# mkshing/e4t-diffusion

Measured on AMD Instinct MI355X. Metric: E4T pretrain images/sec @512px bf16, higher is better.
Workload: dtype bf16

## Files before the change

### e4t-diffusion_amd/csrc/gemm.hip

```cpp
#include "gemm_common.h"

#ifndef E4T_GEMM_PS_DEFAULT
#define E4T_GEMM_PS_DEFAULT 0
#endif
extern "C" __attribute__((visibility("hidden"))) int e4t_launch_gemm_ps(const GemmArgs* p, int conv, int bn, int general, int ncu, hipStream_t st);

namespace {


template <int BM, int BN, int WGM, int WGN, int MODE>
__global__ __launch_bounds__(256) void gemm_kernel(GemmArgs p) {
  constexpr int WM = BM / WGM, WN = BN / WGN;
  constexpr int FM = WM / 32, FN = WN / 32;
  constexpr int NA = BM * (BK / 8) / 256;
  constexpr int NB = BN * (BK / 8) / 256;
  static_assert(WGM * WGN == 4, "4 waves per workgroup");
  static_assert(NA >= 1 && NB >= 1, "tile too small");

  __shared__ __attribute__((aligned(16))) bf16_t smem[(BM + BN) * LDS_LD];
  bf16_t* const As = smem;
  bf16_t* const Bs = smem + BM * LDS_LD;

  const int tid = threadIdx.x;
  const int lane = tid & 63, wave = tid >> 6;
// ... 1033 lines not shown
#pragma unroll
    for (int ks = 0; ks < 2; ++ks)
#pragma unroll
      for (int i = 0; i < 2; ++i)
#pragma unroll
        for (int j = 0; j < 2; ++j)
          acc[mh * 2 + i][j] = __builtin_amdgcn_mfma_f32_32x32x16_bf16(af[i][ks], bfr[j][ks], acc[mh * 2 + i][j], 0, 0, 0);
    __builtin_amdgcn_s_setprio(0);
    __builtin_amdgcn_sched_barrier(0);
    __builtin_amdgcn_s_barrier();
    __builtin_amdgcn_sched_barrier(0);
  };
  auto ktile = [&](auto Bc, auto KXc, auto SPc, auto ALLc, int kt) __attribute__((always_inline)) {
    phase(Bc, I0{}, ALLc, KXc, SPc, kt); phase(Bc, I1{}, ALLc, KXc, SPc, kt); phase(Bc, I2{}, ALLc, KXc, SPc, kt); phase(Bc, I3{}, ALLc, KXc, SPc, kt);
  };

  if (wr == 1) __builtin_amdgcn_s_barrier();
  {
    using YES = std::true_type; using NO = std::false_type;
    int kt = kt_begin;
    for (; kt + 8 <= kt_end; kt += 6) {
      ktile(I0{}, I0{}, I0{}, YES{}, kt);     ktile(I1{}, I1{}, I0{}, YES{}, kt + 1); ktile(I0{}, I2{}, I0{}, YES{}, kt + 2);
      ktile(I1{}, I0{}, I1{}, YES{}, kt + 3); ktile(I0{}, I1{}, I1{}, YES{}, kt + 4); ktile(I1{}, I2{}, I1{}, YES{}, kt + 5);
    }
    if (kt < kt_end) { ktile(I0{}, I0{}, I0{}, NO{}, kt); ktile(I1{}, I1{}, I0{}, NO{}, kt + 1); ktile(I0{}, I2{}, I0{}, NO{}, kt + 2); kt += 3; }
    if (kt < kt_end) { ktile(I1{}, I0{}, I1{}, NO{}, kt); ktile(I0{}, I1{}, I1{}, NO{}, kt + 1); ktile(I1{}, I2{}, I1{}, NO{}, kt + 2); kt += 3; }
  }
  if (wr == 0) __builtin_amdgcn_s_barrier();
  __syncthreads();
  write_tile<64, 64, 2, 2, GENERAL>(p, *(f32x16(*)[2][2])(acc + 0), wave_stage<64, 64>(smem, wave), lane, m0 + wr * 128, n0 + wc * 64);
  __syncthreads();
  write_tile<64, 64, 2, 2, GENERAL>(p, *(f32x16(*)[2][2])(acc + 2), wave_stage<64, 64>(smem, wave), lane, m0 + wr * 128 + 64, n0 + wc * 64);
}
static bool conv_pps_ok(const GemmArgs& p, int batch) {
  static const bool on = CONV_STRIP && getenv("E4T_CONV_NOSTRIP") == nullptr;
  const bool rows = p.Win % 256 == 0 || (p.Win >= 16 && 256 % p.Win == 0 && p.Hin % (256 / p.Win) == 0);
  return on && p.mode == E4T_CONV_S1 && p.chan_major && batch == 1 && rows && p.Wout == p.Win && p.Hout == p.Hin && p.Cin % 64 == 0 &&
         p.K == 9 * p.Cin && p.ktiles_per_split % 3 == 0 && p.M % 256 == 0;
}

template <int MODE, int BN, bool GENERAL>
__global__ __launch_bounds__(512) void gemm_pq_kernel(GemmArgs p) {
  constexpr int BM = 256, HK = 32;
  constexpr int WR = BN == 320 ? 4 : 2, WC = 8 / WR;
  constexpr int WM = BM / WR, WN = BN / WC;
  constexpr int FM = WM / 32, FN = WN / 32;
  constexpr int QA = BM * HK, QB = BN * HK;
  constexpr int HALF = QA + QB, BUF = 2 * HALF;
  constexpr int NBP = BN / 16;
  constexpr int NBJ = (NBP + 7) / 8;
  constexpr int NBLAST = NBP - 8 * (NBJ - 1);
  constexpr int ESTG = 8 * 32 * (WN + 8);
  static_assert(BN == 256 || BN == 320, "tile width");
  static_assert(2 * BUF * 2 <= 160 * 1024 && ESTG <= 2 * BUF, "LDS budget");
  __shared__ __attribute__((aligned(16))) bf16_t smem[2 * BUF];

  const int tid = threadIdx.x;
  const int lane = tid & 63, wave = __builtin_amdgcn_readfirstlane(tid >> 6);
  const int grp = wave >> 2;
  const int wr = wave / WC, wc = wave % WC;
  int tile_x, tile_y;
  xcd_tile(tile_x, tile_y, p.group_m);
  int m0 = tile_y * BM;
  const int n0 = tile_x * BN;
  const int mrows = p.M - m0;
  if (p.panel_rows) m0 = (m0 / p.panel_rows) * p.panel_stride + p.panel_off + m0 % p.panel_rows;

// ... 203 lines not shown
    __builtin_amdgcn_sched_barrier(0);
  };
  using I0 = std::integral_constant<int, 0>; using I1 = std::integral_constant<int, 1>;
  using I2 = std::integral_constant<int, 2>; using I3 = std::integral_constant<int, 3>;

  if (grp == 1) __builtin_amdgcn_s_barrier();
  {
    int kt = kt_begin;
    for (; kt + 2 <= kt_end; kt += 2) {
      phase(I0{}, I0{}, kt); phase(I0{}, I1{}, kt); phase(I0{}, I2{}, kt); phase(I0{}, I3{}, kt);
      phase(I1{}, I0{}, kt + 1); phase(I1{}, I1{}, kt + 1); phase(I1{}, I2{}, kt + 1); phase(I1{}, I3{}, kt + 1);
    }
    if (kt < kt_end) { phase(I0{}, I0{}, kt); phase(I0{}, I1{}, kt); phase(I0{}, I2{}, kt); phase(I0{}, I3{}, kt); }
  }
  if (grp == 0) __builtin_amdgcn_s_barrier();
  __syncthreads();
  if (p.panel_rows) p.M = m0 + min(mrows, BM);
  auto slice = [&](auto Ic) {
    constexpr int i = decltype(Ic)::value;
    write_tile<32, WN, 1, FN, GENERAL>(p, *(f32x16(*)[1][FN])(&acc[i][0]), wave_stage<32, WN>(smem, wave), lane, m0 + wr * WM + i * 32, n0 + wc * WN);
  };
  slice(I0{});
  __syncthreads();
  slice(I1{});
  if constexpr (FM == 4) {
    __syncthreads();
    slice(I2{});
    __syncthreads();
    slice(I3{});
  }
  if constexpr (MODE == 0) {
    if (p.tail_rows) gemm_tail<8, GENERAL>(p, (float*)smem, wave, lane);
  }
}

#ifdef E4T_EXPERIMENTAL
template <int MODE>
__global__ __launch_bounds__(512) void gemm_pt_kernel(GemmArgs p) {
  constexpr int BM = 512, BN = 128, HK = 32;
  constexpr int QA = BM * HK, QB = BN * HK;
  constexpr int HALF = QA + QB;
  constexpr int SMEM = 4 * HALF;
  static_assert(8 * 64 * (64 + 8) <= SMEM, "epilogue staging must fit");
  __shared__ __attribute__((aligned(16))) bf16_t smem[SMEM];

  const int tid = threadIdx.x;
  const int lane = tid & 63, wave = __builtin_amdgcn_readfirstlane(tid >> 6);
  const int wr = wave >> 2, wc = wave & 3;
  int tile_x, tile_y;
  xcd_tile(tile_x, tile_y, p.group_m);
  const int m0 = tile_y * BM, n0 = tile_x * BN;

  const int nkt = p.K / BK;
  const int bz = blockIdx.z / p.splitk, sz = blockIdx.z - bz * p.splitk;
  p.A += bz * p.strideA;
  if (p.A2) p.A2 += bz * p.strideA;
  p.B += bz * p.strideB;
  if (p.bias) p.bias += bz * p.strideBias;
  if (!p.reduce_batch) {
    if (p.flags & E4T_OUT_F32) p.C = (float*)p.C + bz * p.strideC;
    else p.C = (bf16_t*)p.C + bz * p.strideC;
  }
  const int kt_begin = sz * p.ktiles_per_split;
  int kt_end = kt_begin + p.ktiles_per_split;
  if (kt_end > nkt) kt_end = nkt;

// ... 355 lines not shown
    for (int k = 0; k < 8; ++k) {
      float x = v[k] * p.alpha + bi[k] + rb[k];
      if (p.flags & E4T_ACT_GELU) x = gelu_f(x);
      v[k] = x + rs[k];
    }
    *(uint4*)((bf16_t*)p.C + (size_t)row * p.ldc + c8) = pack8(v);
  }
}

__global__ __launch_bounds__(256) void splitk_reduce4f_kernel(GemmArgs p, int nz) {
  const int n4 = p.N >> 2;
  const size_t total = (size_t)p.M * p.N, total4 = (size_t)p.M * n4;
  const int bz = blockIdx.y;
  float* Cf = (float*)p.C + (p.reduce_batch ? 0 : bz * p.strideC);
  const float* ws = p.ws + (size_t)bz * nz * total;
  for (size_t i4 = (size_t)blockIdx.x * 256 + threadIdx.x; i4 < total4; i4 += (size_t)gridDim.x * 256) {
    const int row = (int)(i4 / n4), c4 = (int)(i4 - (size_t)row * n4) * 4;
    const size_t idx = (size_t)row * p.N + c4;
    float4 v = make_float4(0.f, 0.f, 0.f, 0.f);
    for (int z0 = 0; z0 < nz; z0 += 8) {
      float4 t[8];
#pragma unroll
      for (int u = 0; u < 8; ++u) t[u] = *(const float4*)(ws + (size_t)min(z0 + u, nz - 1) * total + idx);
#pragma unroll
      for (int u = 0; u < 8; ++u) {
        const float w = z0 + u < nz ? 1.f : 0.f;
        v.x += t[u].x * w; v.y += t[u].y * w; v.z += t[u].z * w; v.w += t[u].w * w;
      }
    }
    float4* c = (float4*)(Cf + (size_t)row * p.ldc + c4);
    float4 o = make_float4(v.x * p.alpha, v.y * p.alpha, v.z * p.alpha, v.w * p.alpha);
    if (p.flags & E4T_ACCUM) { const float4 a = *c; o.x += a.x; o.y += a.y; o.z += a.z; o.w += a.w; }
    *c = o;
  }
}

struct GemmPlan {
  int tile;
  int stages;
  bool kt32;
  bool general_epi;
  bool buf_ok;
  int tm, tn, gx, gy;
  int splitk, ktiles_per_split;
  unsigned a_bytes, a2_bytes, b_bytes;
};

int device_cu_count() {
  static int ncu = [] {
    int dev = 0, n = 0;
    if (hipGetDevice(&dev) != hipSuccess || hipDeviceGetAttribute(&n, hipDeviceAttributeMultiprocessorCount, dev) != hipSuccess || n <= 0) n = 256;
    return n;
  }();
  return ncu;
}

bool ps_rounds_ok(long long units, int ncu) {
  if (units < ncu) return false;
  const long long rounds = (units + ncu - 1) / ncu;
  return units * 100 >= rounds * ncu * 85;
}

struct SmallGridPlan { int tile, stages, splitk; };
struct SmallGridCand { int tile, stages, tm, tn, occ; float t1, tk, epi; bool general_ok; };
SmallGridPlan small_grid_plan(int M, int N, int nkt, bool conv, bool general, int splitk_req, bool wants_colstats, int ncu) {
  static const SmallGridCand cands[] = {
// ... 1 lines not shown
      {128, 2, 128, 128, 2, 0.875f, 0.544f, 1.08f, true}, {128, 4, 128, 128, 1, 0.596f, 0.544f, 1.08f, false},
      {160, 2, 128, 160, 2, 0.955f, 0.629f, 3.41f, false}, {160, 3, 128, 160, 1, 0.861f, 0.629f, 3.41f, false}};
  static const int splits[] = {1, 2, 3, 4, 6, 8, 12};
  const float launch = 1.6f, pro = 0.945f, red0 = 4.49f, red_bytes_per_us = 4.05e6f, conv_mul = 0.916f, stats_pass = 6.0f;
  SmallGridPlan best = {128, 2, 1};
  float best_t = 1e30f;
  for (const SmallGridCand& c : cands) {
    if (general && !c.general_ok) continue;
    if (c.tile == 160 && N % 160 != 0) continue;
    for (int sk : splits) {
      if (splitk_req > 0 && sk != 1) continue;
      const int s = splitk_req > 0 ? (splitk_req < nkt ? splitk_req : nkt) : sk;
      if (s > 1 && splitk_req <= 0 && (nkt / s < 4 || (double)M * N * s * 4.0 > 256e6)) continue;
      const int kps = cdiv(nkt, s);
      const long long wgs = (long long)cdiv(M, c.tm) * cdiv(N, c.tn) * s;
      const long long per_cu = cdivl(wgs, ncu);
      const long long q = per_cu / c.occ, r = per_cu % c.occ;
      const float full = c.occ > 1 ? c.occ * c.tk : c.t1;
      const float rem = r == 0 ? 0.f : (r == 1 ? c.t1 : (float)r * c.tk);
      float per_kt = (float)q * full + rem;
      if (conv) per_kt *= conv_mul;
      const float rounds = (float)cdivl(per_cu, c.occ);
      float t = launch + rounds * (pro + c.epi) + (float)kps * per_kt;
      if (s > 1) {
        t += red0 + ((float)s * 4.f + 2.f) * (float)M * (float)N / red_bytes_per_us + rounds * c.epi * 0.5f;
        if (wants_colstats) t += stats_pass;
      }
      if (t < best_t) { best_t = t; best = {c.tile, c.stages, s}; }
    }
  }
  return best;
}

GemmPlan plan_gemm(const GemmArgs& p, bool conv, int tile_hint, int splitk_req, int batch) {
  GemmPlan pl;
  const int nkt = cdiv(p.K, BK);
  int stages = 2;
  int model_splitk = 0;
  bool kt32 = false;
  if (tile_hint >= 3000 && tile_hint < 5000) { stages = tile_hint / 1000; tile_hint %= 1000; }
  else if (tile_hint >= 5000 && tile_hint < 6000) { kt32 = true; stages = 4; tile_hint %= 1000; }
  int tile = tile_hint;
#ifndef E4T_EXPERIMENTAL
  if (kt32 && tile != 256) { kt32 = false; stages = 2; }
  if (tile != 64 && tile != 128 && tile != 160) stages = 2;
  if (tile == 256 && !kt32) { kt32 = true; stages = 3; }
  if (tile == 640) tile = 128;
  if (tile == 1128) tile = 128;
  if (tile == 1160) tile = 160;
#endif
  static const bool allow256 = getenv("E4T_GEMM_REGSTAGE") == nullptr;
#ifdef E4T_EXPERIMENTAL
  static const bool auto256 = getenv("E4T_GEMM_AUTO256") != nullptr;
#else
  const bool auto256 = false;
#endif
  const bool r2_rules = false;
  const bool whole_k = p.K % BK == 0 && (!p.A2 || p.K1 % BK == 0);
  const bool ps_ok = allow256 && whole_k && batch == 1 && !p.reduce_batch && splitk_req <= 1;
  if (tile != 64 && tile != 128 && tile != 256 && tile != 160 && tile != 512 && tile != 640 && tile != 1128 && tile != 1160 && tile != 2320) {
    const long long t256 = (long long)cdiv(p.M, 256) * cdiv(p.N, 128) * batch;
    const long long t128 = (long long)cdiv(p.M, 128) * cdiv(p.N, 128) * batch;
    tile = (allow256 && auto256 && t256 >= 256) ? 256 : (t128 >= 256 || (nkt >= 32 && t128 >= 64)) ? 128 : 64;
    if (allow256 && tile == 128 && p.N % 160 == 0 && p.N <= 960 && (long long)cdiv(p.M, 128) * (p.N / 160) * batch >= 128) tile = 160;
    const bool no_pp = false;
    const long long tpp = (long long)cdiv(p.M, 256) * (p.N / 256) * batch;
    if (allow256 && !no_pp && tile == 128 && p.N % 256 == 0 && whole_k && nkt >= (conv ? 16 : (r2_rules ? 32 : 20)) && tpp >= 512) tile = 512;
    if (allow256 && !no_pp && tile == 128 && p.N % 256 == 0 && whole_k && nkt >= 128 && tpp >= 64 && tpp < (r2_rules ? 512 : 256)) tile = 512;
    if (!r2_rules && allow256 && !no_pp && tile == 128 && p.N % 256 == 0 && whole_k && nkt >= 20 && tpp >= 224 && tpp <= 256) tile = 512;
#ifdef E4T_EXPERIMENTAL
    static const bool auto_pt = getenv("E4T_GEMM_PT") != nullptr;
#else
    const bool auto_pt = false;
#endif
    if (auto_pt && allow256 && tile == 128 && p.N % 128 == 0 && p.N % 256 != 0 && p.K % BK == 0 && nkt >= 16 && !p.A2 &&
        (long long)cdiv(p.M, 512) * (p.N / 128) * batch >= 512) tile = 640;
    const bool general = (p.flags & E4T_ACT_GELU) || (p.rowbias && p.rows_per_batch % 32 != 0);
    if (!r2_rules && allow256 && tile == 128 && !general && p.N % 160 == 0 && p.N > 960 && nkt >= 20 &&
        (long long)cdiv(p.M, 128) * (p.N / 160) * batch >= 1024) tile = 160;
    if (!r2_rules && allow256 && tile == 128 && !general && (p.N % 128 == 0 || p.N < 128) &&
        (long long)cdiv(p.M, 256) * cdiv(p.N, 128) * batch >= 768) { tile = 256; kt32 = true; stages = 3; }
    const bool no_pq = false;
    if (!r2_rules && !no_pq && allow256 && batch == 1 && (!general || !conv) && whole_k && p.N % 320 == 0) {
      const long long t320 = (long long)cdiv(p.M, 256) * (p.N / 320);
      const int ncu = device_cu_count();
      const double eff = (double)t320 / (double)(cdivl(t320, ncu) * ncu);
      if (t320 >= ncu && ((nkt >= 20 && eff >= 0.75) || (nkt >= 10 && eff >= 0.99) || (nkt >= 5 && p.N == 320 && eff >= 0.99))) {
        tile = 2320; kt32 = false; stages = 2;
      }
    }
#ifdef E4T_EXPERIMENTAL
    static const int auto_ps = getenv("E4T_GEMM_PS") ? atoi(getenv("E4T_GEMM_PS")) : E4T_GEMM_PS_DEFAULT;
#else
    const int auto_ps = 0;
#endif
    if (auto_ps && ps_ok && (tile == 128 || tile == 160)) {
      const int ncu = device_cu_count();
      const long long rows = cdiv(p.M, 256);
      if (p.N % 160 == 0 && ps_rounds_ok(rows * (p.N / 160), ncu)) tile = 1160;
      else if ((p.N % 128 == 0 || p.N < 128) && ps_rounds_ok(rows * cdiv(p.N, 128), ncu)) tile = 1128;
    }
    const bool no_model = false;
    if (!no_model && allow256 && (tile == 64 || tile == 128 || tile == 160) && batch == 1 && !p.reduce_batch && !p.panel_rows) {
      const SmallGridPlan sg = small_grid_plan(p.M, p.N, nkt, conv, general, splitk_req, p.colstats != nullptr, device_cu_count());
      tile = sg.tile; stages = sg.stages; model_splitk = sg.splitk;
    }
  }
  const bool general_epi = (p.flags & E4T_ACT_GELU) || (p.rowbias && p.rows_per_batch % 32 != 0);
  if (general_epi) { if (!(tile == 64 && stages == 3)) stages = 2; kt32 = false; if (tile == 256 || tile == 640) tile = 128; }
  if (kt32 && tile != 128 && tile != 64 && tile != 256) kt32 = false;
  if (kt32 && tile == 256) stages = 3;
  if (tile == 256 && !allow256) tile = 128;
  if (tile == 160 && !allow256) tile = 128;
  if (tile == 640 && (!allow256 || p.A2)) tile = 128;
  if ((tile == 1128 || tile == 1160) && !ps_ok) tile = tile == 1160 && p.N % 160 == 0 ? 160 : 128;
  if (tile == 2320 && !allow256) tile = 128;
  if (tile == 2320 && general_epi && conv) tile = p.N % 160 == 0 ? 160 : 128;
  if (p.panel_rows && !(tile == 2320 && allow256)) tile = (p.N % 320 == 0 && whole_k && !conv) ? 2320 : tile;
  bool buf_ok = true;
  {
    const unsigned long long lim = 0xFFFF0000ull;
    unsigned long long ab, a2b = 0, bb = ((unsigned long long)(p.N - 1) * p.ldb + p.K) * 2;
    if (conv) ab = (unsigned long long)((long long)p.M / ((long long)p.Hout * p.Wout)) * p.Hin * p.Win * p.Cin * 2;
    else {
      const unsigned long long last = p.panel_rows ? (unsigned long long)((p.M - 1) / p.panel_rows) * p.panel_stride + p.panel_off + (p.M - 1) % p.panel_rows : (unsigned long long)(p.M - 1);
      ab = (last * p.lda + p.K1) * 2;
      if (p.A2) a2b = (last * p.lda2 + (p.K - p.K1)) * 2;
    }
    buf_ok = ab < lim && a2b < lim && bb < lim;
    if (tile == 512 && (!allow256 || !buf_ok || !whole_k)) tile = 128;
    if (tile == 2320 && (!buf_ok || !whole_k || p.N % 320 != 0)) tile = 128;
    if (tile == 640 && (!buf_ok || p.K % BK != 0)) tile = 128;
    pl.a_bytes = (unsigned)(buf_ok ? ab : 0); pl.a2_bytes = (unsigned)(buf_ok ? a2b : 0); pl.b_bytes = (unsigned)(buf_ok ? bb : 0);
    if (!buf_ok && tile != 64) { tile = 128; kt32 = false; stages = 2; }
  }
  const int tm = tile == 160 ? 128 : (tile == 512 || tile >= 1000 ? 256 : (tile == 640 ? 512 : tile));
  const int tn = tile == 256 ? 128 : (tile == 512 ? 256 : (tile == 640 ? 128 : (tile >= 1000 ? tile % 1000 : tile)));
  const bool pingpong = tile == 512 || tile == 2320;
  const int gx = cdiv(p.N, tn), gy = cdiv(p.M, tm);
  int splitk = splitk_req;
  if (tile >= 1000 && tile < 2000) splitk = 1;
  if (p.panel_rows) splitk = 1;
  if (splitk <= 0 && model_splitk > 0 && (tile == 64 || tile == 128 || tile == 160)) splitk = model_splitk;
  if (splitk <= 0) {
    splitk = 1;
    const long long tiles = (long long)gx * gy * batch;
    if (pingpong && (tiles < 256 || !r2_rules)) {
      if (tiles < 256) {
        splitk = (int)(256 / tiles);
        if (splitk > nkt / 16) splitk = nkt / 16;
      }
    } else if (tile >= 128 && tiles < 512 && nkt >= 32) {
      splitk = (int)((tiles <= 256 ? 512 : 1024) / tiles);
      if (splitk > 8) splitk = 8;
      if (splitk > nkt / 16) splitk = nkt / 16;
      if (tiles > 256 && nkt < 128) splitk = 1;
    } else if (tile == 64 && tiles < 256 && nkt >= 32) {
      splitk = (int)((512 + tiles - 1) / tiles);
      if (splitk > nkt / 16) splitk = nkt / 16;
    }
    if (splitk < 1) splitk = 1;
  }
  if (splitk > nkt) splitk = nkt;
  pl.ktiles_per_split = cdiv(nkt, splitk);
  pl.splitk = cdiv(nkt, pl.ktiles_per_split);
  pl.tile = tile; pl.stages = stages; pl.kt32 = kt32; pl.general_epi = general_epi; pl.buf_ok = buf_ok;
  pl.tm = tm; pl.tn = tn; pl.gx = gx; pl.gy = gy;
  return pl;
}

size_t plan_workspace_bytes(const GemmPlan& pl, const GemmArgs& p, int batch) {
  return (pl.splitk > 1 || p.reduce_batch) ? (size_t)pl.splitk * batch * p.M * p.N * sizeof(float) : 0;
}

// ... 34 lines not shown
                 (unsigned long long)p.a_bytes + (unsigned long long)(p.Win + 1) * p.Cin * 2 < 0xFFFF0000ull;
  static const bool allow256 = getenv("E4T_GEMM_REGSTAGE") == nullptr;
  (void)allow256;
  const bool need_ws = splitk > 1 || p.reduce_batch;
  const size_t need = (size_t)splitk * batch * p.M * p.N * sizeof(float);
  if (need_ws && (p.ws == nullptr || ws_bytes < need)) {
    if (splitk_req > 1 || p.reduce_batch)
      E4T_FAIL(-12, "gemm: split-K=%d batch=%d needs %zu workspace bytes, have %zu", splitk, batch, need, ws_bytes);
    splitk = 1;
    p.ktiles_per_split = nkt;
  }
  if (!(splitk > 1 || p.reduce_batch)) p.ws = nullptr;
  p.splitk = splitk;
  p.group_m = 8;
  p.fast_epi = !(p.flags & (E4T_OUT_F32 | E4T_ACCUM | E4T_RES_F32)) && p.N % 8 == 0 && p.ldc % 8 == 0 && ((uintptr_t)p.C & 15) == 0 &&
               (p.strideC % 8 == 0) && (!p.residual || (p.ldr % 8 == 0 && ((uintptr_t)p.residual & 15) == 0));
  p.fast_f32 = (p.flags & E4T_OUT_F32) && !(p.flags & E4T_ACCUM) && !p.rowbias && (!p.residual || (p.flags & E4T_RES_F32)) &&
               (!(p.flags & E4T_ACT_GELU) || general_epi);
  if (p.colstats && (p.ws || !p.fast_epi || p.M % 32 != 0 || batch != 1)) p.colstats = nullptr;
  const int stats_written = p.colstats != nullptr;
  const bool vec8 = p.ws && !(p.flags & (E4T_OUT_F32 | E4T_ACCUM | E4T_RES_F32)) && p.N % 8 == 0 && p.ldc % 8 == 0 && ((uintptr_t)p.C & 15) == 0 &&
                    p.strideC % 8 == 0 && (!p.residual || (p.ldr % 8 == 0 && ((uintptr_t)p.residual & 15) == 0)) &&
                    (!p.bias || (((uintptr_t)p.bias & 15) == 0 && p.strideBias % 4 == 0)) &&
                    (!p.rowbias || (((uintptr_t)p.rowbias & 15) == 0 && p.ldrb % 4 == 0)) && ((uintptr_t)p.ws & 15) == 0;
  dim3 grid(gx, gy, splitk * batch), block(256);
  static const bool use_dma = getenv("E4T_GEMM_REGSTAGE") == nullptr;
  if (e4t_launch_log_enabled()) {
    const double osz = (p.flags & E4T_OUT_F32) ? 4.0 : 2.0;
    const double a_el = conv ? (double)(p.M / ((long long)p.Hout * p.Wout)) * p.Hin * p.Win * p.Cin : (double)p.M * p.K * batch;
    double by = 2.0 * a_el + 2.0 * (double)p.N * p.K * (p.strideB || batch == 1 ? batch : 1) + osz * (double)p.M * p.N * (p.reduce_batch ? 1 : batch);
    if (p.residual) by += ((p.flags & E4T_RES_F32) ? 4.0 : 2.0) * (double)p.M * p.N;
    if (p.flags & E4T_ACCUM) by += osz * (double)p.M * p.N;
    const char* sym = !(use_dma && buf_ok) ? "gemm_kernel"
                      : tile == 512 && conv && conv_pps_ok(p, batch) ? (general_epi ? "gemm_pps_kernel<true>" : "gemm_pps_kernel<false>")
                      : tile == 512 ? (general_epi ? (conv ? (p.chan_major ? "gemm_pp_kernel<1, true, true>" : "gemm_pp_kernel<1, true, false>") : "gemm_pp_kernel<0, true, false>")
                                                   : (conv ? (p.chan_major ? "gemm_pp_kernel<1, false, true>" : "gemm_pp_kernel<1, false, false>") : "gemm_pp_kernel<0, false, false>"))
                      : tile == 640 ? (conv ? "gemm_pt_kernel<1>" : "gemm_pt_kernel<0>")
                      : tile == 256 && !kt32 ? (conv ? "gemm_dma_kernel<256, 128, 4, 2, 1, 3, false, 64>" : "gemm_dma_kernel<256, 128, 4, 2, 0, 3, false, 64>")
                      : tile == 256 ? (conv ? (conv_strip_ok(p, splitk, batch) ? "conv_strip_kernel<2>" : "gemm_dma_kernel<256, 128, 4, 2, 1, 3, false, 32>")
                                            : "gemm_dma_kernel<256, 128, 4, 2, 0, 3, false, 32>")
                      : nullptr;
    char symbuf[64];
    if (!sym && tile >= 2000) {
      snprintf(symbuf, sizeof(symbuf), "gemm_pq_kernel<%d, %d, %s>", conv ? 1 : 0, tile - 2000, general_epi ? "true" : "false");
      sym = symbuf;
    }
    if (!sym && tile >= 1000) {
      snprintf(symbuf, sizeof(symbuf), "gemm_ps_kernel<%d, %d, %s>", conv ? 1 : 0, tile - 1000, general_epi ? "true" : "false");
      sym = symbuf;
    }
    if (!sym) {
      snprintf(symbuf, sizeof(symbuf), "gemm_dma_kernel<%d, %d, %d, %d, %d, %d, %s, %d>", tile == 64 ? 64 : 128, tile == 160 ? 160 : tile, tile == 64 ? 2 : 4,
               tile == 160 ? 1 : 2, conv ? 1 : 0, stages, general_epi ? "true" : "false", kt32 ? 32 : 64);
      sym = symbuf;
    }
    if (conv) E4T_LOG_LAUNCH("%s|conv mode%d %dx%d->%dx%d Cin%d Cout%d M%d splitk%d|%.0f|%.0f", sym, p.mode, p.Hin, p.Win, p.Hout, p.Wout, p.Cin, p.N,
                             p.M, splitk, by, 2.0 * p.M * p.N * (double)p.K);
    else E4T_LOG_LAUNCH("%s|gemm M%d N%d K%d batch%d splitk%d flags%d|%.0f|%.0f", sym, m_all, p.N, p.K, batch, splitk, p.flags,
                        by + (double)tail * (2.0 * p.K + (osz + (p.residual ? ((p.flags & E4T_RES_F32) ? 4.0 : 2.0) : 0.0)) * p.N), 2.0 * m_all * p.N * (double)p.K * batch);
    if (p.ws) E4T_LOG_LAUNCH("%s|M%d N%d nz%d|%.0f|0", vec8 ? "splitk_reduce8_kernel" : reduce4f_ok(p) ? "splitk_reduce4f_kernel" : "splitk_reduce_kernel",
                             p.M, p.N, p.reduce_batch ? splitk * batch : splitk, 4.0 * (double)p.M * p.N * splitk * batch + osz * (double)p.M * p.N);
  }
  if (p.panel_rows && !(use_dma && buf_ok && tile == 2320 && splitk == 1 && !p.ws))
    E4T_FAIL(-22, "gemm: row panels need the 256 x 320 ping-pong tile (N %% 320 == 0, K %% 64 == 0, no split-K); the plan chose tile %d", tile);
  if (use_dma && buf_ok) {
    if (tile == 2320) {
      block = dim3(512);
      if (conv) hipLaunchKernelGGL((gemm_pq_kernel<1, 320, false>), grid, block, 0, st, p);
      else if (general_epi) hipLaunchKernelGGL((gemm_pq_kernel<0, 320, true>), grid, block, 0, st, p);
      else hipLaunchKernelGGL((gemm_pq_kernel<0, 320, false>), grid, block, 0, st, p);
#ifdef E4T_EXPERIMENTAL
    } else if (tile >= 1000) {
      static const bool ps_pre = getenv("E4T_PS_PRE") == nullptr || atoi(getenv("E4T_PS_PRE")) != 0;
      p.ps_pre = ps_pre && p.fast_epi && nkt >= 2 && (!p.rowbias || p.rows_per_batch % 256 == 0);
      const int rc = e4t_launch_gemm_ps(&p, conv ? 1 : 0, tile - 1000, general_epi ? 1 : 0, device_cu_count(), st);
      if (rc < 0) return rc;
#endif
    } else if (tile == 512) {
      block = dim3(512);
      if (conv && conv_pps_ok(p, batch)) {
        if (general_epi) hipLaunchKernelGGL((gemm_pps_kernel<true>), grid, block, 0, st, p);
        else hipLaunchKernelGGL((gemm_pps_kernel<false>), grid, block, 0, st, p);
      } else if (general_epi) {
        if (conv && p.chan_major) hipLaunchKernelGGL((gemm_pp_kernel<1, true, true>), grid, block, 0, st, p);
        else if (conv) hipLaunchKernelGGL((gemm_pp_kernel<1, true>), grid, block, 0, st, p);
        else hipLaunchKernelGGL((gemm_pp_kernel<0, true>), grid, block, 0, st, p);
      } else {
#ifdef E4T_EXPERIMENTAL
        static const bool strip256 = getenv("E4T_CONV_STRIP256") != nullptr && atoi(getenv("E4T_CONV_STRIP256")) != 0;
        if (conv && strip256 && conv_strip_ok(p, splitk, batch)) hipLaunchKernelGGL(conv_strip_kernel<4>, grid, dim3(1024), 0, st, p);
        else
#endif
        if (conv && p.chan_major) hipLaunchKernelGGL((gemm_pp_kernel<1, false, true>), grid, block, 0, st, p);
        else if (conv) hipLaunchKernelGGL((gemm_pp_kernel<1>), grid, block, 0, st, p);
        else hipLaunchKernelGGL((gemm_pp_kernel<0>), grid, block, 0, st, p);
      }
#ifdef E4T_EXPERIMENTAL
    } else if (tile == 640) {
      block = dim3(512);
      if (conv) hipLaunchKernelGGL((gemm_pt_kernel<1>), grid, block, 0, st, p);
      else hipLaunchKernelGGL((gemm_pt_kernel<0>), grid, block, 0, st, p);
#endif
    } else if (tile == 256 && kt32) {
      block = dim3(512);
      if (conv && conv_strip_ok(p, splitk, batch)) hipLaunchKernelGGL(conv_strip_kernel<2>, grid, block, 0, st, p);
      else if (conv) hipLaunchKernelGGL((gemm_dma_kernel<256, 128, 4, 2, 1, 3, false, 32>), grid, block, 0, st, p);
      else hipLaunchKernelGGL((gemm_dma_kernel<256, 128, 4, 2, 0, 3, false, 32>), grid, block, 0, st, p);
#ifdef E4T_EXPERIMENTAL
    } else if (tile == 256) {
      block = dim3(512);
      if (conv) hipLaunchKernelGGL((gemm_dma_kernel<256, 128, 4, 2, 1, 3>), grid, block, 0, st, p);
      else hipLaunchKernelGGL((gemm_dma_kernel<256, 128, 4, 2, 0, 3>), grid, block, 0, st, p);
#endif
// ... 243 lines not shown
```

Before: 161.7.

## Add strip-reuse implicit-GEMM conv kernel for 256x320 ping-pong tile

Adds gemm_pqs_kernel, a 256x320 ping-pong conv kernel that loads one haloed input row strip per ky into LDS and reuses it across the three kx taps, instead of gathering a full im2col A tile per k-tile. It is dispatched for stride-1 channel-major 3x3 convs that meet the strip conditions when the plan picks tile 2320. The goal is to cut global/LDS traffic for the A operand. In exchange it adds a complex hand-tuned vmcnt wait schedule and always uses the non-general epilogue.

```diff
diff --git a/e4t-diffusion_amd/csrc/gemm.hip b/e4t-diffusion_amd/csrc/gemm.hip
--- a/e4t-diffusion_amd/csrc/gemm.hip
+++ b/e4t-diffusion_amd/csrc/gemm.hip
@@ -1089,7 +1089,7 @@
   __syncthreads();
   write_tile<64, 64, 2, 2, GENERAL>(p, *(f32x16(*)[2][2])(acc + 2), wave_stage<64, 64>(smem, wave), lane, m0 + wr * 128 + 64, n0 + wc * 64);
 }
-static bool conv_pps_ok(const GemmArgs& p, int batch) {
+static bool conv_strip256_ok(const GemmArgs& p, int batch) {
   static const bool on = CONV_STRIP && getenv("E4T_CONV_NOSTRIP") == nullptr;
   const bool rows = p.Win % 256 == 0 || (p.Win >= 16 && 256 % p.Win == 0 && p.Hin % (256 / p.Win) == 0);
   return on && p.mode == E4T_CONV_S1 && p.chan_major && batch == 1 && rows && p.Wout == p.Win && p.Hout == p.Hin && p.Cin % 64 == 0 &&
@@ -1359,6 +1359,187 @@
   if constexpr (MODE == 0) {
     if (p.tail_rows) gemm_tail<8, GENERAL>(p, (float*)smem, wave, lane);
   }
+}
+
+#ifndef CONV_STRIP_PQ
+#define CONV_STRIP_PQ 1
+#endif
+__global__ __launch_bounds__(512) void gemm_pqs_kernel(GemmArgs p) {
+  constexpr int BM = 256, BN = 320, HK = 32;
+  constexpr int WM = 64, WN = 160, FM = 2, FN = 5;
+  constexpr int QB = BN * HK;
+  constexpr int HSTRIP = 320 * HK;
+  constexpr int A_EL = 4 * HSTRIP;
+  constexpr int SMEM = A_EL + 4 * QB;
+  static_assert(8 * 32 * (WN + 8) <= SMEM && 2 * SMEM <= 160 * 1024, "LDS budget");
+  __shared__ __attribute__((aligned(16))) bf16_t smem[SMEM];
+
+  const int tid = threadIdx.x;
+  const int lane = tid & 63, wave = __builtin_amdgcn_readfirstlane(tid >> 6);
+  const int grp = wave >> 2;
+  const int wr = wave >> 1, wc = wave & 1;
+  int tile_x, tile_y;
+  xcd_tile(tile_x, tile_y, p.group_m);
+  const int m0 = tile_y * BM, n0 = tile_x * BN;
+
+  const int nkt = p.K / BK;
+  const int sz = blockIdx.z;
+  const int kt_begin = sz * p.ktiles_per_split;
+  int kt_end = kt_begin + p.ktiles_per_split;
+  if (kt_end > nkt) kt_end = nkt;
+
+  const int hw = p.Hin * p.Win;
+  const int ib = m0 / hw, rem = m0 - ib * hw, y = rem / p.Win, x0 = rem - y * p.Win;
+  const int segw = p.Win < 256 ? p.Win : 256, SW = segw + 2, nrows = 256 / segw;
+  const __amdgpu_buffer_rsrc_t rs_a = cm_rsrc(p);
+  const __amdgpu_buffer_rsrc_t rs_b = uniform_rsrc(p.B, p.b_bytes);
+  constexpr unsigned OOB = 0xFFFF0000u;
+  const int drow = lane >> 2, dslot = lane & 3;
+  const bool a3 = wave >= 4;
+  unsigned a_vo[3];
+  int a_inv[3];
+#pragma unroll
+  for (int i = 0; i < 3; ++i) {
+    const int j = 16 * (i < 2 ? wave + 8 * i : wave + 12) + drow;
+    const int ry = j / SW, xs = j - ry * SW, ix = x0 - 1 + xs;
+    const bool ok = ry < nrows && ix >= 0 && ix < p.Win;
+    a_vo[i] = (unsigned)(((ry * p.Win + xs) * p.Cin + (dslot ^ ((j >> 2) & 3)) * 8) * 2);
+    int m = 0;
+#pragma unroll
+    for (int ky = 0; ky < 3; ++ky) {
+      const int iy = y + ry + ky - 1;
+      if (!(ok && iy >= 0 && iy < p.Hin)) m |= 1 << ky;
+    }
+    a_inv[i] = m;
+  }
+  constexpr int NBJ = 3, NBLAST = 4;
+  unsigned b_vo[NBJ];
+#pragma unroll
+  for (int j = 0; j < NBJ; ++j) {
+    const int r = (wave + 8 * j) * 16 + drow;
+    const int gn = n0 + r;
+    b_vo[j] = (r < BN && gn < p.N) ? (unsigned)(((size_t)gn * p.ldb + (dslot ^ ((r >> 2) & 3)) * 8) * 2) : OOB;
+  }
+  CmWalk wb;
+  wb.init(kt_begin, BK);
+  int b_so = 0;
+  int a_ky = (kt_begin % 9) / 3, a_chb = (kt_begin / 9) * BK * 2;
+  auto issue_b = [&](bool hi, bf16_t* dst) __attribute__((always_inline)) {
+    if (!hi) b_so = cm_b_so(p, wb);
+    else b_so = __builtin_amdgcn_readfirstlane(b_so + HK * 2);
+#pragma unroll
+    for (int j = 0; j < NBJ; ++j)
+      if (j < NBJ - 1 || wave < NBLAST) buf_dma16(rs_b, b_vo[j], b_so, dst + ((wave + 8 * j) * 16) * HK);
+    if (hi) wb.next(BK);
+  };
+  auto issue_strip_piece = [&](auto Ic, bf16_t* dst_lo) __attribute__((always_inline)) {
+    constexpr int i = decltype(Ic)::value;
+    if (i < 2 || a3) {
+      const int iy = y + a_ky - 1;
+      const int so = __builtin_amdgcn_readfirstlane((int)((((long long)ib * p.Hin + iy + 1) * p.Win + x0) * p.Cin * 2) + a_chb);
+      const unsigned vo = a_vo[i] | (unsigned)__builtin_amdgcn_sbfe(a_inv[i], (unsigned)a_ky, 1u);
+      const int q = i < 2 ? wave + 8 * i : wave + 12;
+      buf_dma16(rs_a, vo, so, dst_lo + q * 16 * HK);
+      buf_dma16(rs_a, vo, so + HK * 2, dst_lo + HSTRIP + q * 16 * HK);
+    }
+    if (i == 2 && ++a_ky == 3) { a_ky = 0; a_chb += BK * 2; }
+  };
+
+  f32x16 acc[FM][FN];
+#pragma unroll
+  for (int i = 0; i < FM; ++i)
+#pragma unroll
+    for (int j = 0; j < FN; ++j)
+#pragma unroll
+      for (int r = 0; r < 16; ++r) acc[i][j][r] = 0.f;
+
+  const int frow = lane & 31, fhi = lane >> 5;
+  int a_off[3][FM][2], b_off[2];
+#pragma unroll
+  for (int ks = 0; ks < 2; ++ks) {
+#pragma unroll
+    for (int kx = 0; kx < 3; ++kx)
+#pragma unroll
+      for (int i = 0; i < FM; ++i) {
+        const int o = wr * WM + i * 32 + frow;
+        const int r = (o / segw) * SW + o % segw + kx;
+        a_off[kx][i][ks] = r * HK + (((ks * 2 + fhi) ^ ((r >> 2) & 3)) * 8);
+      }
+    const int r = wc * WN + frow;
+    b_off[ks] = r * HK + (((ks * 2 + fhi) ^ ((r >> 2) & 3)) * 8);
+  }
+  using I0 = std::integral_constant<int, 0>; using I1 = std::integral_constant<int, 1>;
+  using I2 = std::integral_constant<int, 2>; using I3 = std::integral_constant<int, 3>;
+  bf16_t* const Bq = smem + A_EL;
+  issue_strip_piece(I0{}, smem);
+  issue_strip_piece(I1{}, smem);
+  issue_strip_piece(I2{}, smem);
+  issue_b(false, Bq);
+  issue_b(true, Bq + QB);
+  if (kt_begin + 1 < kt_end) issue_b(false, Bq + 2 * QB);
+  wait_vmcnt<0>();
+  __builtin_amdgcn_s_barrier();
+
+  auto phase = [&](auto Bc, auto Pc, auto ALLc, auto KXc, auto SPc, int kt) {
+    constexpr int bb = decltype(Bc)::value, ph = decltype(Pc)::value, KX = decltype(KXc)::value, SP = decltype(SPc)::value;
+    constexpr bool ALL = decltype(ALLc)::value;
+    constexpr int kh = ph >> 1, ks = ph & 1;
+    constexpr int G = 4 * KX + ph;
+    const bf16_t* const qa = smem + (2 * SP + kh) * HSTRIP;
+    const bf16_t* const qb = Bq + (2 * bb + kh) * QB;
+    bf16x8 af[FM], bfr[FN];
+#pragma unroll
+    for (int i = 0; i < FM; ++i) af[i] = *(const bf16x8*)(qa + a_off[KX][i][ks]);
+#pragma unroll
+    for (int j = 0; j < FN; ++j) bfr[j] = *(const bf16x8*)(qb + b_off[ks] + j * 32 * HK);
+    bool staged = true;
+    bf16_t* const next_strip = smem + 2 * (SP ^ 1) * HSTRIP;
+    if (ph == 1)      { staged = ALL || kt + 1 < kt_end; if (staged) issue_b(true, Bq + (2 * (bb ^ 1) + 1) * QB); }
+    else if (ph == 3) { staged = ALL || kt + 2 < kt_end; if (staged) issue_b(false, Bq + (2 * bb + 0) * QB); }
+    else if (G == 2)  { staged = ALL || kt + 3 < kt_end; if (staged) issue_strip_piece(I0{}, next_strip); }
+    else if (G == 4)  { staged = ALL || kt + 2 < kt_end; if (staged) issue_strip_piece(I1{}, next_strip); }
+    else if (G == 6)  { staged = ALL || kt + 2 < kt_end; if (staged) issue_strip_piece(I2{}, next_strip); }
+    constexpr int NW_HI = G <= 1 ? 6 : G <= 3 ? 8 : G <= 5 ? 10 : G <= 7 ? 8 : 6;
+    constexpr int NW_LO = G <= 1 ? 4 : G <= 3 ? 6 : G <= 7 ? 8 : G <= 9 ? 6 : 4;
+    if (ALL || staged) {
+      if (wave < NBLAST) wait_vmcnt<NW_HI>(); else wait_vmcnt<NW_LO>();
+    } else {
+      wait_vmcnt<0>();
+    }
+    __builtin_amdgcn_sched_barrier(0);
+    __builtin_amdgcn_s_barrier();
+    __builtin_amdgcn_sched_barrier(0);
+    __builtin_amdgcn_s_setprio(1);
+#pragma unroll
+    for (int i = 0; i < FM; ++i)
+#pragma unroll
+      for (int j = 0; j < FN; ++j)
+        acc[i][j] = __builtin_amdgcn_mfma_f32_32x32x16_bf16(af[i], bfr[j], acc[i][j], 0, 0, 0);
+    __builtin_amdgcn_s_setprio(0);
+    __builtin_amdgcn_sched_barrier(0);
+    __builtin_amdgcn_s_barrier();
+    __builtin_amdgcn_sched_barrier(0);
+  };
+  auto ktile = [&](auto Bc, auto KXc, auto SPc, auto ALLc, int kt) __attribute__((always_inline)) {
+    phase(Bc, I0{}, ALLc, KXc, SPc, kt); phase(Bc, I1{}, ALLc, KXc, SPc, kt); phase(Bc, I2{}, ALLc, KXc, SPc, kt); phase(Bc, I3{}, ALLc, KXc, SPc, kt);
+  };
+
+  if (grp == 1) __builtin_amdgcn_s_barrier();
+  {
+    using YES = std::true_type; using NO = std::false_type;
+    int kt = kt_begin;
+    for (; kt + 8 <= kt_end; kt += 6) {
+      ktile(I0{}, I0{}, I0{}, YES{}, kt);     ktile(I1{}, I1{}, I0{}, YES{}, kt + 1); ktile(I0{}, I2{}, I0{}, YES{}, kt + 2);
+      ktile(I1{}, I0{}, I1{}, YES{}, kt + 3); ktile(I0{}, I1{}, I1{}, YES{}, kt + 4); ktile(I1{}, I2{}, I1{}, YES{}, kt + 5);
+    }
+    if (kt < kt_end) { ktile(I0{}, I0{}, I0{}, NO{}, kt); ktile(I1{}, I1{}, I0{}, NO{}, kt + 1); ktile(I0{}, I2{}, I0{}, NO{}, kt + 2); kt += 3; }
+    if (kt < kt_end) { ktile(I1{}, I0{}, I1{}, NO{}, kt); ktile(I0{}, I1{}, I1{}, NO{}, kt + 1); ktile(I1{}, I2{}, I1{}, NO{}, kt + 2); kt += 3; }
+  }
+  if (grp == 0) __builtin_amdgcn_s_barrier();
+  __syncthreads();
+  write_tile<32, WN, 1, FN, false>(p, *(f32x16(*)[1][FN])(&acc[0][0]), wave_stage<32, WN>(smem, wave), lane, m0 + wr * WM, n0 + wc * WN);
+  __syncthreads();
+  write_tile<32, WN, 1, FN, false>(p, *(f32x16(*)[1][FN])(&acc[1][0]), wave_stage<32, WN>(smem, wave), lane, m0 + wr * WM + 32, n0 + wc * WN);
 }
 
 #ifdef E4T_EXPERIMENTAL
@@ -2055,9 +2236,10 @@
     if (p.residual) by += ((p.flags & E4T_RES_F32) ? 4.0 : 2.0) * (double)p.M * p.N;
     if (p.flags & E4T_ACCUM) by += osz * (double)p.M * p.N;
     const char* sym = !(use_dma && buf_ok) ? "gemm_kernel"
-                      : tile == 512 && conv && conv_pps_ok(p, batch) ? (general_epi ? "gemm_pps_kernel<true>" : "gemm_pps_kernel<false>")
+                      : tile == 512 && conv && conv_strip256_ok(p, batch) ? (general_epi ? "gemm_pps_kernel<true>" : "gemm_pps_kernel<false>")
                       : tile == 512 ? (general_epi ? (conv ? (p.chan_major ? "gemm_pp_kernel<1, true, true>" : "gemm_pp_kernel<1, true, false>") : "gemm_pp_kernel<0, true, false>")
                                                    : (conv ? (p.chan_major ? "gemm_pp_kernel<1, false, true>" : "gemm_pp_kernel<1, false, false>") : "gemm_pp_kernel<0, false, false>"))
+                      : tile == 2320 && conv && CONV_STRIP_PQ && conv_strip256_ok(p, batch) ? "gemm_pqs_kernel"
                       : tile == 640 ? (conv ? "gemm_pt_kernel<1>" : "gemm_pt_kernel<0>")
                       : tile == 256 && !kt32 ? (conv ? "gemm_dma_kernel<256, 128, 4, 2, 1, 3, false, 64>" : "gemm_dma_kernel<256, 128, 4, 2, 0, 3, false, 64>")
                       : tile == 256 ? (conv ? (conv_strip_ok(p, splitk, batch) ? "conv_strip_kernel<2>" : "gemm_dma_kernel<256, 128, 4, 2, 1, 3, false, 32>")
@@ -2089,7 +2271,8 @@
   if (use_dma && buf_ok) {
     if (tile == 2320) {
       block = dim3(512);
-      if (conv) hipLaunchKernelGGL((gemm_pq_kernel<1, 320, false>), grid, block, 0, st, p);
+      if (conv && CONV_STRIP_PQ && conv_strip256_ok(p, batch)) hipLaunchKernelGGL(gemm_pqs_kernel, grid, block, 0, st, p);
+      else if (conv) hipLaunchKernelGGL((gemm_pq_kernel<1, 320, false>), grid, block, 0, st, p);
       else if (general_epi) hipLaunchKernelGGL((gemm_pq_kernel<0, 320, true>), grid, block, 0, st, p);
       else hipLaunchKernelGGL((gemm_pq_kernel<0, 320, false>), grid, block, 0, st, p);
 #ifdef E4T_EXPERIMENTAL
@@ -2101,7 +2284,7 @@
 #endif
     } else if (tile == 512) {
       block = dim3(512);
-      if (conv && conv_pps_ok(p, batch)) {
+      if (conv && conv_strip256_ok(p, batch)) {
         if (general_epi) hipLaunchKernelGGL((gemm_pps_kernel<true>), grid, block, 0, st, p);
         else hipLaunchKernelGGL((gemm_pps_kernel<false>), grid, block, 0, st, p);
       } else if (general_epi) {
```

Result: no change. 162.4, median of 6 (+0.4%).

## Add weight-resident persistent GEMM kernel for small-K, N=640/960 linear layers

Applied to the files above, without the earlier changes.

Adds a persistent GEMM kernel for small K (at most five 64-wide chunks) and N of 640 or 960. Each workgroup keeps a 160-column slab of the weight matrix resident in LDS and streams 128-row A tiles through a three-slot DMA ring. Bias, residual add and column statistics are fused into an epilogue that overlaps with the next tile's loads. The planner routes eligible non-conv GEMMs to it automatically, removing repeated weight reloads and per-tile launch overhead. The cost is one workgroup per CU, a fixed grid mapping that assumes 8 XCDs, and a narrower set of supported shapes.

```diff
diff --git a/e4t-diffusion_amd/csrc/gemm.hip b/e4t-diffusion_amd/csrc/gemm.hip
--- a/e4t-diffusion_amd/csrc/gemm.hip
+++ b/e4t-diffusion_amd/csrc/gemm.hip
@@ -1780,6 +1780,183 @@
     float4 o = make_float4(v.x * p.alpha, v.y * p.alpha, v.z * p.alpha, v.w * p.alpha);
     if (p.flags & E4T_ACCUM) { const float4 a = *c; o.x += a.x; o.y += a.y; o.z += a.z; o.w += a.w; }
     *c = o;
+  }
+}
+
+typedef unsigned ws_u32x4 __attribute__((__vector_size__(16)));
+typedef unsigned ws_u32x2 __attribute__((__vector_size__(8)));
+constexpr int WS_BM = 128, WS_SN = 160, WS_NKC = 5, WS_NSLOT = 3, WS_ELD = 40;
+
+template <bool RES, bool CST>
+__global__ __launch_bounds__(256, 1) void gemm_ws_kernel(GemmArgs p) {
+  constexpr int FN = WS_SN / 32;
+  constexpr int SLAB = WS_SN * BK, SLOT = WS_BM * BK, STG = 32 * WS_ELD;
+  constexpr int EPI_OPS = 2 * FN + (RES ? 2 * FN : 0) + (CST ? FN : 0);
+  __shared__ __attribute__((aligned(16))) bf16_t slab[WS_NKC * SLAB];
+  __shared__ __attribute__((aligned(16))) bf16_t ring[WS_NSLOT * SLOT];
+  __shared__ __attribute__((aligned(16))) bf16_t stage[4 * STG];
+  static_assert(sizeof(slab) + sizeof(ring) + sizeof(stage) <= 160 * 1024, "LDS budget");
+  const int tid = threadIdx.x;
+  const int lane = tid & 63, wave = __builtin_amdgcn_readfirstlane(tid >> 6);
+  bf16_t* const stg = stage + wave * STG;
+
+  const int nslab = p.N / WS_SN;
+  const int xcd = blockIdx.x & 7, j8 = blockIdx.x >> 3;
+  const int gpx = (gridDim.x >> 3) / nslab, ngrp = 8 * gpx;
+  const int n0 = (j8 % nslab) * WS_SN, grp = xcd * gpx + j8 / nslab;
+  const int ntile_all = (p.M + WS_BM - 1) / WS_BM;
+  const int t_begin = (int)((long long)grp * ntile_all / ngrp), t_end = (int)((long long)(grp + 1) * ntile_all / ngrp);
+  const int nkc = p.K / BK;
+  const int nch = (t_end - t_begin) * nkc;
+  if (nch <= 0) return;
+
+  const __amdgpu_buffer_rsrc_t rs_a = uniform_rsrc(p.A, p.a_bytes);
+  const __amdgpu_buffer_rsrc_t rs_b = uniform_rsrc(p.B, p.b_bytes);
+  const __amdgpu_buffer_rsrc_t rs_c = uniform_rsrc(p.C, (unsigned)(((unsigned long long)(p.M - 1) * p.ldc + p.N) * 2));
+  const __amdgpu_buffer_rsrc_t rs_r = uniform_rsrc(RES ? p.residual : p.C, RES ? (unsigned)(((unsigned long long)(p.M - 1) * p.ldr + p.N) * 2) : 0u);
+  const __amdgpu_buffer_rsrc_t rs_s = uniform_rsrc(CST ? (const void*)p.colstats : p.C, CST ? (unsigned)((unsigned long long)(p.M >> 5) * p.N * 8) : 0u);
+  constexpr unsigned OOB = 0xFFFF0000u;
+  const int lrow = lane >> 3, lslot = lane & 7;
+  auto swz = [](int r) { return (r >> 1) & 7; };
+  const int frow = lane & 31, fhi = lane >> 5;
+
+  float bv[FN];
+#pragma unroll
+  for (int j = 0; j < FN; ++j) {
+    bv[j] = p.bias ? p.bias[n0 + j * 32 + frow] : 0.f;
+    asm volatile("" : "+v"(bv[j]));
+  }
+
+#pragma unroll
+  for (int i = 0; i < WS_SN / 8 / 4; ++i) {
+    const int r = (wave + 4 * i) * 8 + lrow;
+    const unsigned vo = (unsigned)(((size_t)(n0 + r) * p.ldb + (lslot ^ swz(r)) * 8) * 2);
+    for (int kc = 0; kc < nkc; ++kc)
+      buf_dma16(rs_b, vo, __builtin_amdgcn_readfirstlane(kc * BK * 2), slab + kc * SLAB + (wave + 4 * i) * 512);
+  }
+  int is_t = t_begin, is_kc = 0, is_slot = 0;
+  unsigned a_vo[4];
+  auto issue_chunk = [&]() __attribute__((always_inline)) {
+    if (is_kc == 0) {
+#pragma unroll
+      for (int i = 0; i < 4; ++i) {
+        const int r = (wave * 4 + i) * 8 + lrow, gr = is_t * WS_BM + r;
+        a_vo[i] = gr < p.M ? (unsigned)(((size_t)gr * p.lda + (lslot ^ swz(r)) * 8) * 2) : OOB;
+      }
+    }
+    const int so = __builtin_amdgcn_readfirstlane(is_kc * BK * 2);
+#pragma unroll
+    for (int i = 0; i < 4; ++i) buf_dma16(rs_a, a_vo[i], so, ring + is_slot * SLOT + (wave * 4 + i) * 512);
+    if (++is_kc == nkc) { is_kc = 0; ++is_t; }
+    is_slot = is_slot == WS_NSLOT - 1 ? 0 : is_slot + 1;
+  };
+  issue_chunk();
+  if (nch > 1) issue_chunk();
+
+  int a_off[4], b_off[FN][4];
+#pragma unroll
+  for (int ks = 0; ks < 4; ++ks) {
+    const int ra = wave * 32 + frow;
+    a_off[ks] = ra * BK + (((ks * 2 + fhi) ^ swz(ra)) * 8);
+#pragma unroll
+    for (int j = 0; j < FN; ++j) {
+      const int rb = j * 32 + frow;
+      b_off[j][ks] = rb * BK + (((ks * 2 + fhi) ^ swz(rb)) * 8);
+    }
+  }
+  f32x16 acc[FN];
+#pragma unroll
+  for (int j = 0; j < FN; ++j)
+#pragma unroll
+    for (int r = 0; r < 16; ++r) acc[j][r] = 0.f;
+
+  int kc = 0, slot = 0, t = t_begin;
+  for (int c = 0; c < nch; ++c) {
+    const bool next = c + 1 < nch;
+    const bool epi = (c >= 2 && (c - 2) % nkc == nkc - 1) || (c >= 1 && (c - 1) % nkc == nkc - 1);
+    if (next && epi) wait_vmcnt<4 + EPI_OPS>();
+    else if (next) wait_vmcnt<4>();
+    else if (epi) wait_vmcnt<EPI_OPS>();
+    else wait_vmcnt<0>();
+    loop_barrier();
+    if (c + 2 < nch) issue_chunk();
+#ifndef E4T_WS_PROBE
+    {
+      const bf16_t* As = ring + slot * SLOT;
+      const bf16_t* Bs = slab + kc * SLAB;
+      bf16x8 af[2], bfr[2][FN];
+      af[0] = *(const bf16x8*)(As + a_off[0]);
+#pragma unroll
+      for (int j = 0; j < FN; ++j) bfr[0][j] = *(const bf16x8*)(Bs + b_off[j][0]);
+#pragma unroll
+      for (int ks = 0; ks < 4; ++ks) {
+        const int cu = ks & 1, nx = cu ^ 1;
+        if (ks + 1 < 4) {
+          af[nx] = *(const bf16x8*)(As + a_off[ks + 1]);
+#pragma unroll
+          for (int j = 0; j < FN; ++j) bfr[nx][j] = *(const bf16x8*)(Bs + b_off[j][ks + 1]);
+        }
+#pragma unroll
+        for (int j = 0; j < FN; ++j) acc[j] = __builtin_amdgcn_mfma_f32_32x32x16_bf16(af[cu], bfr[cu][j], acc[j], 0, 0, 0);
+      }
+    }
+#endif
+    if (kc == nkc - 1) {
+      const int mw = t * WS_BM + wave * 32;
+      ws_u32x4 rres[2 * FN];
+      if constexpr (RES) {
+#pragma unroll
+        for (int u = 0; u < 2 * FN; ++u) {
+          const int id = (u & 1) * 64 + lane, rl = id >> 2, cch = id & 3;
+          const int row = mw + rl, col = n0 + (u >> 1) * 32 + cch * 8;
+          rres[u] = __builtin_amdgcn_raw_buffer_load_b128(rs_r, row < p.M ? (unsigned)(((size_t)row * p.ldr + col) * 2) : OOB, 0, 0);
+        }
+      }
+#pragma unroll
+      for (int j = 0; j < FN; ++j) {
+        const float add = bv[j] + 0.f;
+#pragma unroll
+        for (int r = 0; r < 16; ++r) {
+          const int rl = (r & 3) + 8 * (r >> 2) + 4 * fhi;
+          stg[rl * WS_ELD + frow] = f2bf(acc[j][r] * p.alpha + add);
+        }
+        __builtin_amdgcn_sched_barrier(0);
+#pragma unroll
+        for (int h = 0; h < 2; ++h) {
+          const int id = h * 64 + lane, rl = id >> 2, cch = id & 3;
+          uint4 v = *(const uint4*)(stg + rl * WS_ELD + cch * 8);
+          if constexpr (RES) {
+            float a[8], b[8];
+            unpack8(v, a);
+            unpack8(__builtin_bit_cast(uint4, rres[j * 2 + h]), b);
+#pragma unroll
+            for (int k = 0; k < 8; ++k) a[k] += b[k];
+            v = pack8(a);
+            if constexpr (CST) *(uint4*)(stg + rl * WS_ELD + cch * 8) = v;
+          }
+          const int row = mw + rl, col = n0 + j * 32 + cch * 8;
+          __builtin_amdgcn_raw_buffer_store_b128(__builtin_bit_cast(ws_u32x4, v), rs_c, row < p.M ? (unsigned)(((size_t)row * p.ldc + col) * 2) : OOB, 0, 0);
+        }
+        if constexpr (CST) {
+          float sm = 0.f, sq = 0.f;
+#pragma unroll 8
+          for (int r = 0; r < 32; ++r) {
+            const float x = bf2f(stg[r * WS_ELD + frow]);
+            sm += x; sq += x * x;
+          }
+          const unsigned so = (lane < 32 && mw < p.M) ? (unsigned)((((size_t)(mw >> 5)) * p.N + n0 + j * 32 + frow) * 8) : OOB;
+          __builtin_amdgcn_raw_buffer_store_b64(ws_u32x2{__float_as_uint(sm), __float_as_uint(sq)}, rs_s, so, 0, 0);
+        }
+        __builtin_amdgcn_sched_barrier(0);
+      }
+#pragma unroll
+      for (int j = 0; j < FN; ++j)
+#pragma unroll
+        for (int r = 0; r < 16; ++r) acc[j][r] = 0.f;
+      ++t;
+    }
+    if (++kc == nkc) kc = 0;
+    slot = slot == WS_NSLOT - 1 ? 0 : slot + 1;
   }
 }
 
@@ -1847,6 +2024,21 @@
   return best;
 }
 
+int ws_plan(const GemmArgs& p, bool conv, int batch, int splitk_req, int ncu) {
+  if (conv || batch != 1 || p.reduce_batch || p.A2 || p.panel_rows || splitk_req > 1 || p.rowbias) return 0;
+  if (p.flags & (E4T_OUT_F32 | E4T_ACCUM | E4T_RES_F32 | E4T_ACT_GELU)) return 0;
+  if (p.K % BK != 0 || p.K < 2 * BK || p.K > WS_NKC * BK || p.N % WS_SN != 0 || p.N > 8 * WS_SN) return 0;
+  if (p.lda % 8 || p.ldb % 8 || p.ldc % 8 || (((uintptr_t)p.A | (uintptr_t)p.B | (uintptr_t)p.C) & 15)) return 0;
+  if (p.residual && (p.ldr % 8 || ((uintptr_t)p.residual & 15))) return 0;
+  const int nslab = p.N / WS_SN, gpx = (ncu / 8) / nslab;
+  if (gpx < 1 || (long long)cdiv(p.M, WS_BM) < 4LL * 8 * gpx) return 0;
+  const unsigned long long lim = 0xFFFF0000ull;
+  const unsigned long long ab = ((unsigned long long)(p.M - 1) * p.lda + p.K) * 2, bb = ((unsigned long long)(p.N - 1) * p.ldb + p.K) * 2;
+  const unsigned long long cb = ((unsigned long long)(p.M - 1) * p.ldc + p.N) * 2, rb = p.residual ? ((unsigned long long)(p.M - 1) * p.ldr + p.N) * 2 : 0;
+  if (ab >= lim || bb >= lim || cb >= lim || rb >= lim || (unsigned long long)(p.M / 32) * p.N * 8 >= lim) return 0;
+  return 8 * gpx * nslab;
+}
+
 GemmPlan plan_gemm(const GemmArgs& p, bool conv, int tile_hint, int splitk_req, int batch) {
   GemmPlan pl;
   const int nkt = cdiv(p.K, BK);
@@ -1873,7 +2065,10 @@
   const bool r2_rules = false;
   const bool whole_k = p.K % BK == 0 && (!p.A2 || p.K1 % BK == 0);
   const bool ps_ok = allow256 && whole_k && batch == 1 && !p.reduce_batch && splitk_req <= 1;
-  if (tile != 64 && tile != 128 && tile != 256 && tile != 160 && tile != 512 && tile != 640 && tile != 1128 && tile != 1160 && tile != 2320) {
+  const int ws_grid = ws_plan(p, conv, batch, splitk_req, device_cu_count());
+  if (tile == 6160 && ws_grid == 0) tile = 0;
+  if (tile != 64 && tile != 128 && tile != 256 && tile != 160 && tile != 512 && tile != 640 && tile != 1128 && tile != 1160 && tile != 2320 &&
+      tile != 6160) {
     const long long t256 = (long long)cdiv(p.M, 256) * cdiv(p.N, 128) * batch;
     const long long t128 = (long long)cdiv(p.M, 128) * cdiv(p.N, 128) * batch;
     tile = (allow256 && auto256 && t256 >= 256) ? 256 : (t128 >= 256 || (nkt >= 32 && t128 >= 64)) ? 128 : 64;
@@ -1920,6 +2115,7 @@
       const SmallGridPlan sg = small_grid_plan(p.M, p.N, nkt, conv, general, splitk_req, p.colstats != nullptr, device_cu_count());
       tile = sg.tile; stages = sg.stages; model_splitk = sg.splitk;
     }
+    if (ws_grid > 0 && (p.N == 640 || p.N == 960)) { tile = 6160; kt32 = false; stages = 2; model_splitk = 0; }
   }
   const bool general_epi = (p.flags & E4T_ACT_GELU) || (p.rowbias && p.rows_per_batch % 32 != 0);
   if (general_epi) { if (!(tile == 64 && stages == 3)) stages = 2; kt32 = false; if (tile == 256 || tile == 640) tile = 128; }
@@ -1949,12 +2145,13 @@
     pl.a_bytes = (unsigned)(buf_ok ? ab : 0); pl.a2_bytes = (unsigned)(buf_ok ? a2b : 0); pl.b_bytes = (unsigned)(buf_ok ? bb : 0);
     if (!buf_ok && tile != 64) { tile = 128; kt32 = false; stages = 2; }
   }
-  const int tm = tile == 160 ? 128 : (tile == 512 || tile >= 1000 ? 256 : (tile == 640 ? 512 : tile));
+  if (tile == 6160 && (ws_grid == 0 || !buf_ok)) tile = 128;
+  const int tm = tile == 160 || tile == 6160 ? 128 : (tile == 512 || tile >= 1000 ? 256 : (tile == 640 ? 512 : tile));
   const int tn = tile == 256 ? 128 : (tile == 512 ? 256 : (tile == 640 ? 128 : (tile >= 1000 ? tile % 1000 : tile)));
   const bool pingpong = tile == 512 || tile == 2320;
-  const int gx = cdiv(p.N, tn), gy = cdiv(p.M, tm);
+  const int gx = tile == 6160 ? ws_grid : cdiv(p.N, tn), gy = tile == 6160 ? 1 : cdiv(p.M, tm);
   int splitk = splitk_req;
-  if (tile >= 1000 && tile < 2000) splitk = 1;
+  if ((tile >= 1000 && tile < 2000) || tile == 6160) splitk = 1;
   if (p.panel_rows) splitk = 1;
   if (splitk <= 0 && model_splitk > 0 && (tile == 64 || tile == 128 || tile == 160)) splitk = model_splitk;
   if (splitk <= 0) {
@@ -2064,6 +2261,10 @@
                                             : "gemm_dma_kernel<256, 128, 4, 2, 0, 3, false, 32>")
                       : nullptr;
     char symbuf[64];
+    if (!sym && tile == 6160) {
+      snprintf(symbuf, sizeof(symbuf), "gemm_ws_kernel<%s, %s>", p.residual ? "true" : "false", p.colstats ? "true" : "false");
+      sym = symbuf;
+    }
     if (!sym && tile >= 2000) {
       snprintf(symbuf, sizeof(symbuf), "gemm_pq_kernel<%d, %d, %s>", conv ? 1 : 0, tile - 2000, general_epi ? "true" : "false");
       sym = symbuf;
@@ -2087,7 +2288,14 @@
   if (p.panel_rows && !(use_dma && buf_ok && tile == 2320 && splitk == 1 && !p.ws))
     E4T_FAIL(-22, "gemm: row panels need the 256 x 320 ping-pong tile (N %% 320 == 0, K %% 64 == 0, no split-K); the plan chose tile %d", tile);
   if (use_dma && buf_ok) {
-    if (tile == 2320) {
+    if (tile == 6160) {
+      if (p.ws || !p.fast_epi || p.splitk != 1) E4T_FAIL(-22, "gemm: the weight-resident kernel needs a single-pass bf16 epilogue");
+      block = dim3(256);
+      if (p.residual && p.colstats) hipLaunchKernelGGL((gemm_ws_kernel<true, true>), grid, block, 0, st, p);
+      else if (p.residual) hipLaunchKernelGGL((gemm_ws_kernel<true, false>), grid, block, 0, st, p);
+      else if (p.colstats) hipLaunchKernelGGL((gemm_ws_kernel<false, true>), grid, block, 0, st, p);
+      else hipLaunchKernelGGL((gemm_ws_kernel<false, false>), grid, block, 0, st, p);
+    } else if (tile == 2320) {
       block = dim3(512);
       if (conv) hipLaunchKernelGGL((gemm_pq_kernel<1, 320, false>), grid, block, 0, st, p);
       else if (general_epi) hipLaunchKernelGGL((gemm_pq_kernel<0, 320, true>), grid, block, 0, st, p);
```

Measured after the change: 167.1 before, 166.8 after (median of 6 runs). No clear change (-0.2%).
